# datasciencetoolkit/NextGP.jl

Measured on AMD Instinct MI355X. Metric: gibbs_iterations_per_sec, higher is better.
Workload: dtype f64; 1 GPU; single-trait Gibbs sweep, N=50000 individuals x P=600000 SNPs, marker sets BayesPR(200000) + BayesPR(200000) + BayesPR(200000), fp32 panel in HBM (BASELINE.json configs[3]: multi-breed random regression = three BayesPR marker sets of 200,000 SNPs); N=50000, P=600000, chains=1, panel_dtype=f32, accumulate_dtype=f64

## Files before the change

include/nextgp_hip.h:

```cpp
#ifndef NEXTGP_HIP_H
#define NEXTGP_HIP_H

#include <stdint.h>

#ifdef __cplusplus
extern "C" {
#endif

#define NGP_ABI_VERSION 4

#define NGP_OK 0
#define NGP_ERR_ARG (-1)
#define NGP_ERR_STATE (-2)
#define NGP_ERR_HIP (-3)
#define NGP_ERR_NOMEM (-4)
#define NGP_ERR_NODEVICE (-5)
#define NGP_ERR_DEBUG (-6)

#define NGP_METHOD_BAYESPR 0
#define NGP_METHOD_BAYESB 1
#define NGP_METHOD_BAYESC 2
#define NGP_METHOD_BAYESR 3
#define NGP_METHOD_TUPLE 4
#define NGP_METHOD_BAYESLV 5
// ... 94 lines not shown

int32_t ngp_draws_indexed(ngp_handle *h, uint64_t iter, uint64_t kind, uint64_t index0, int32_t what, double p1, double p2,
                          int64_t n, double *out);
int32_t ngp_eval_math(ngp_handle *h, int32_t which, const double *in, int64_t n, double *out);

int32_t ngp_set_streamer(ngp_handle *h, int32_t variant);
int32_t ngp_get_streamer(ngp_handle *h, int32_t *variant, int32_t *gemv_chains);

int32_t ngp_set_max_shards(ngp_handle *h, int32_t max_shards);
int32_t ngp_shards_for_chains(ngp_handle *h, int32_t chains, int32_t *max_shards);
int32_t ngp_share_panel(ngp_handle *h, ngp_handle *owner);
int32_t ngp_shards_for_pass(ngp_handle *h, int32_t chains, int32_t *max_shards);
#define NGP_STORAGE_F32 0
#define NGP_STORAGE_U8 1
int32_t ngp_set_storage(ngp_handle *h, int32_t storage);
int32_t ngp_get_storage(ngp_handle *h, int32_t *storage, double *means, int64_t P);

int32_t ngp_debug_set_mode(ngp_handle *h, int32_t mode);
int32_t ngp_debug_set_knob(ngp_handle *h, int32_t knob);

int32_t ngp_set_posterior_sums(ngp_handle *h, const double *sum_beta, const double *sum_beta2, const double *sum_delta,
                               const double *sum_varBeta, const double *sum_pi, double sum_varE, double sum_b, int64_t nKept);
int32_t ngp_save_snapshot(ngp_handle *h, const char *path);
int32_t ngp_load_snapshot(ngp_handle *h, const char *path);

int32_t ngp_set_trace_loci(ngp_handle *h, const int64_t *loci, int64_t n, int64_t n_varBeta);
int32_t ngp_get_trace_ext(ngp_handle *h, double *beta_tr, double *varBeta_tr, double *pi_tr, int64_t n);

int32_t ngp_allreduce_posterior(ngp_handle **hs, int32_t n);
int32_t ngp_run_many(ngp_handle **hs, int32_t n, int64_t niter);

int32_t ngp_set_sample_file(ngp_handle *h, const char *path);
int32_t ngp_get_census(ngp_handle *h, uint64_t *out, int64_t n, int64_t *grid, int64_t *retries, int32_t *exclusive);
int32_t ngp_debug_fail_census(ngp_handle *h, int64_t iteration);
int32_t ngp_debug_set_virtual_device(ngp_handle *h, int32_t vdev);
int32_t ngp_debug_throw(ngp_handle *h, int32_t kind);

int32_t ngp_add_marker_set_lv(ngp_handle *h, int64_t col0, int64_t ncol, double varBeta0, const double *C, int64_t ld, int32_t ncov,
                              double varZeta0, int32_t est_mode, double est_fraction, const double *zeta0, const double *lhs0,
                              const double *rhs0, int32_t *set_id);
int32_t ngp_get_lv_state(ngp_handle *h, int32_t set_id, double *c, double *sum_c, double *varZeta, double *sum_varZeta, double *zeta,
                         double *iCpC, int64_t *trapped);
int32_t ngp_set_lv_state(ngp_handle *h, int32_t set_id, const double *c, const double *sum_c, double varZeta, double sum_varZeta,
                         const double *zeta);

int32_t ngp_grm_begin(ngp_handle *h, int64_t N, int32_t method);
int32_t ngp_grm_columns_f64(ngp_handle *h, const double *M, int64_t ncol, int64_t ld);
int32_t ngp_grm_columns_f32(ngp_handle *h, const float *M, int64_t ncol, int64_t ld);
int32_t ngp_grm_columns_u8(ngp_handle *h, const uint8_t *M, int64_t ncol, int64_t ld);
int32_t ngp_grm_end(ngp_handle *h);
int32_t ngp_grm_get(ngp_handle *h, double *G_out);
int32_t ngp_grm_invert(ngp_handle *h);
int32_t ngp_add_random_set_dense(ngp_handle *h, const int32_t *level, int64_t q, const double *K, ngp_handle *k_src, int32_t k_src_set,
                                 double df, double scale, double varU0, int32_t *set_id);
int32_t ngp_set_records(ngp_handle *h, int64_t N);

#ifdef __cplusplus
}
#endif
#endif
```

nextgp.jl_amd/_lib.py:

```python
import ctypes as C
import os

import numpy as np

_HERE = os.path.dirname(os.path.abspath(__file__))
LIB_PATH = os.environ.get("NGP_HIP_LIB") or os.path.join(_HERE, "libnextgp_hip.so")

METHOD_BAYESPR, METHOD_BAYESB, METHOD_BAYESC, METHOD_BAYESR, METHOD_TUPLE, METHOD_BAYESLV = 0, 1, 2, 3, 4, 5
LV_MAXCOV, LV_WORDS = 16, 17


def _sample_header(f, path):
    magic = f.read(8)
    if magic not in (b"NGPSMP01", b"NGPSMP02", b"NGPSMP03"):
        raise NextGPHipError(f"not a sample file: {path}")
    P, nvb, nsets, nfix, ncls, rec = (int(v) for v in np.frombuffer(f.read(48), dtype=np.int64))
    sets = [dict(zip(("method", "K", "col0", "ncol", "nvb", "tk"), np.frombuffer(f.read(48), dtype=np.int64).tolist())) for _ in range(nsets)]
    rq = []
    if magic in (b"NGPSMP02", b"NGPSMP03"):
        nr = int(np.frombuffer(f.read(8), dtype=np.int64)[0])
        rq = np.frombuffer(f.read(8 * nr), dtype=np.int64).tolist()
    lv = []
    if magic == b"NGPSMP03":
        nl = int(np.frombuffer(f.read(8), dtype=np.int64)[0])
# ... 73 lines not shown
    return col0 + 64 * (l // Lb) + k * (l % Lb) + np.arange(k, dtype=np.int64)[None, :]


def tuple_span(nloc, k):
    Lb = 64 // k
    nblk = (nloc + Lb - 1) // Lb
    return 64 * (nblk - 1) + k * (nloc - Lb * (nblk - 1))


def tuple_panel(sets):
    k, (N, nloc) = len(sets), sets[0].shape
    out = np.zeros((N, tuple_span(nloc, k)), dtype=sets[0].dtype, order="F")
    cols = tuple_columns(0, nloc, k)
    for m, X in enumerate(sets):
        out[:, cols[:, m]] = X
    return out

SYMBOLS = [
    "ngp_abi_version", "ngp_create", "ngp_destroy", "ngp_last_error", "ngp_set_panel_f64", "ngp_set_panel_f32", "ngp_set_panel_u8",
    "ngp_begin_panel", "ngp_panel_columns_f64", "ngp_panel_columns_f32", "ngp_panel_columns_u8", "ngp_end_panel",
    "ngp_generate_panel", "ngp_get_layout", "ngp_get_mpm", "ngp_get_gram", "ngp_xbeta", "ngp_add_marker_set", "ngp_set_y",
    "ngp_set_residual_prior", "ngp_set_intercept", "ngp_set_schedule", "ngp_run", "ngp_get_state", "ngp_set_state",
    "ngp_get_trace", "ngp_get_posterior_sums", "ngp_posterior_len", "ngp_export_posterior_device", "ngp_sweep_set", "ngp_sweep_set_dev",
    "ngp_get_timing", "ngp_profile_iteration", "ngp_draws_indexed", "ngp_eval_math", "ngp_configure", "ngp_get_config", "ngp_debug_stamps", "ngp_set_near_lags", "ngp_get_near_lags",
    "ngp_set_streamer", "ngp_get_streamer", "ngp_set_storage", "ngp_get_storage", "ngp_set_max_shards", "ngp_shards_for_chains", "ngp_run_many", "ngp_write_panel_file", "ngp_read_panel_header", "ngp_load_panel_file", "ngp_debug_set_mode", "ngp_debug_set_knob", "ngp_set_posterior_sums", "ngp_save_snapshot", "ngp_load_snapshot",
    "ngp_set_trace_loci", "ngp_get_trace_ext", "ngp_allreduce_posterior", "ngp_add_marker_set_r", "ngp_get_class_state", "ngp_set_class_state", "ngp_add_fixed_set", "ngp_get_fixed", "ngp_set_fixed", "ngp_debug_throw", "ngp_get_census", "ngp_debug_set_virtual_device", "ngp_debug_fail_census", "ngp_add_marker_set_tuple", "ngp_share_panel", "ngp_shards_for_pass", "ngp_set_sample_file",
    "ngp_set_chain_form", "ngp_get_chain_form", "ngp_get_setup_timing", "ngp_set_residual_weights", "ngp_get_residual_weights",
    "ngp_add_random_set", "ngp_get_random", "ngp_set_random", "ngp_sample_random_set",
    "ngp_add_marker_set_lv", "ngp_get_lv_state", "ngp_set_lv_state",
    "ngp_grm_begin", "ngp_grm_columns_f64", "ngp_grm_columns_f32", "ngp_grm_columns_u8", "ngp_grm_end", "ngp_grm_get", "ngp_grm_invert",
    "ngp_add_random_set_dense", "ngp_set_records",
    "ngp_set_random_schedule", "ngp_get_random_schedule", "ngp_pedigree_ainv",
    "ngp_add_random_set_tuple", "ngp_get_random_tuple", "ngp_set_random_tuple", "ngp_sample_random_set_tuple",
]

_lib = None


class NextGPHipError(RuntimeError):
    pass


def load():
    global _lib
    if _lib is None:
        if not os.path.exists(LIB_PATH):
            raise NextGPHipError(
                f"{LIB_PATH} is missing: build it with `python -c 'import __graft_entry__ as g; g.build()'` "
                "(hipcc --offload-arch=gfx950). There is no CPU fallback.")
        L = C.CDLL(LIB_PATH)
        L.ngp_last_error.restype = C.c_char_p
        L.ngp_last_error.argtypes = [C.c_void_p]
        _lib = L
    return _lib


def _p(a, t):
    return a.ctypes.data_as(C.POINTER(t)) if a is not None else None


def write_panel_file(path, G, bits=8):
    G = np.asfortranarray(G, dtype=np.uint8)
    rc = load().ngp_write_panel_file(str(path).encode(), _p(G, C.c_uint8), C.c_int64(G.shape[0]), C.c_int64(G.shape[1]),
                                     C.c_int64(G.shape[0]), C.c_int32(bits))
    if rc != 0:
        raise NextGPHipError(f"ngp_write_panel_file failed ({rc}): path not writable, or codes above 2 with bits=2")
# ... 536 lines not shown
    def set_posterior_sums(self, ps):
        a = {k: np.ascontiguousarray(ps[k], dtype=np.float64) for k in ("sum_beta", "sum_beta2", "sum_delta", "sum_varBeta", "sum_pi")}
        self._chk(self.L.ngp_set_posterior_sums(self.h, _p(a["sum_beta"], C.c_double), _p(a["sum_beta2"], C.c_double),
                                                _p(a["sum_delta"], C.c_double), _p(a["sum_varBeta"], C.c_double), _p(a["sum_pi"], C.c_double),
                                                C.c_double(ps["sum_varE"]), C.c_double(ps["sum_b"]), C.c_int64(ps["nKept"])))

    def set_sample_file(self, path):
        self._chk(self.L.ngp_set_sample_file(self.h, None if path is None else os.fsencode(path)))

    def save_snapshot(self, path):
        self._chk(self.L.ngp_save_snapshot(self.h, os.fsencode(path)))

    def load_snapshot(self, path):
        self._chk(self.L.ngp_load_snapshot(self.h, os.fsencode(path)))

    def set_trace_loci(self, loci, n_varBeta=0):
        loci = np.ascontiguousarray(loci, dtype=np.int64)
        self._chk(self.L.ngp_set_trace_loci(self.h, _p(loci, C.c_int64) if len(loci) else None, C.c_int64(len(loci)), C.c_int64(n_varBeta)))
        self.ntl, self.ntvb = len(loci), n_varBeta

    def get_trace_ext(self, n):
        bt = np.empty((n, max(self.ntl, 1))); vt = np.empty((n, max(self.ntvb, 1))); pt = np.empty((n, max(self.nsets, 1)))
        self._chk(self.L.ngp_get_trace_ext(self.h, _p(bt, C.c_double), _p(vt, C.c_double), _p(pt, C.c_double), C.c_int64(n)))
        return dict(beta=bt[:, :self.ntl], varBeta=vt[:, :self.ntvb], pi=pt[:, :self.nsets])

    def census(self):
        g, r, e = C.c_int64(), C.c_int64(), C.c_int32()
        self._chk(self.L.ngp_get_census(self.h, None, C.c_int64(0), C.byref(g), C.byref(r), C.byref(e)))
        tb = np.zeros(g.value, dtype=np.uint64)
        self._chk(self.L.ngp_get_census(self.h, _p(tb, C.c_uint64), C.c_int64(g.value), None, None, None))
        return dict(grid=g.value, retries=r.value, exclusive=bool(e.value), xcc=(tb >> np.uint64(32)).astype(np.int64) - 1,
                    hw_id=(tb & np.uint64(0xFFFFFFFF)).astype(np.int64))

    def debug_fail_census(self, iteration):
        self._chk(self.L.ngp_debug_fail_census(self.h, C.c_int64(iteration)))

    def debug_set_virtual_device(self, vdev):
        self._chk(self.L.ngp_debug_set_virtual_device(self.h, C.c_int32(vdev)))

    @staticmethod
    def allreduce_posterior(samplers):
        L = samplers[0].L
        arr = (C.c_void_p * len(samplers))(*[s.h for s in samplers])
        samplers[0]._chk(L.ngp_allreduce_posterior(arr, C.c_int32(len(samplers))))

    @staticmethod
    def run_many(samplers, niter):
        L = samplers[0].L
        arr = (C.c_void_p * len(samplers))(*[s.h for s in samplers])
        rc = L.ngp_run_many(arr, C.c_int32(len(samplers)), C.c_int64(niter))
        if rc != 0:
            msgs = [(s.L.ngp_last_error(s.h) or b"").decode() for s in samplers]
            raise NextGPHipError(f"libnextgp_hip error {rc}: " + " | ".join(m for m in msgs if m))

    def profile_iteration(self):
        ms, by = C.c_double(), C.c_double()
        n = C.c_int64()
        self._chk(self.L.ngp_profile_iteration(self.h, C.byref(ms), C.byref(n), C.byref(by)))
        return dict(avg_ms=ms.value, launches=n.value, bytes_per_launch=by.value)

    def draws_indexed(self, it, kind, index0, what, n, p1=0.0, p2=0.0):
        out = np.empty(n)
        self._chk(self.L.ngp_draws_indexed(self.h, C.c_uint64(it), C.c_uint64(kind), C.c_uint64(index0), C.c_int32(what),
                                           C.c_double(p1), C.c_double(p2), C.c_int64(n), _p(out, C.c_double)))
        return out

# ... 6 lines not shown
```

nextgp.jl_amd/csrc/ngp_api.hip:

```cpp
#include <hip/hip_runtime.h>

#include <dlfcn.h>

#include <algorithm>
#include <chrono>
#include <cmath>
#include <cstdio>
#include <cstdlib>
#include <condition_variable>
#include <cstddef>
#include <cstring>
#include <array>
#include <deque>
#include <map>
#include <memory>
#include <mutex>
#include <queue>
#include <string>
#include <thread>
#include <vector>

#include "../../include/nextgp_hip.h"
#include "ngp_kernels.h"
#include "ngp_random.h"
// ... 807 lines not shown
        HCHK(hipMemcpy(h->mm.d_tseg_len, h->h_tseg_len.data(), h->h_tseg_len.size() * sizeof(int32_t), hipMemcpyHostToDevice));
        HCHK(hipMemcpy(h->mm.d_tseg_set, h->h_tseg_set.data(), h->h_tseg_set.size() * sizeof(int32_t), hipMemcpyHostToDevice));
    }
    h->tables_dirty = false;
    return NGP_OK;
}

bool is_kept(const ngp_handle *h, int64_t it) {
    if (it < h->burnIn + h->thin || it > h->chainLength) return false;
    return ((it - h->burnIn) % h->thin) == 0;
}

void fill_sweep_args(ngp_handle *h, int64_t tb0, int64_t tb1, SweepArgs &A) {
    const int R = (int)h->plan.R, S = (int)h->plan.S;
    A.tiles = h->pm->tiles; A.ycorr = h->cm.d_ycorr; A.gramx = h->pm->gramx;
    const bool tf = wants_tinv(h) && h->cm.tinv_blocks == h->NBLK;
    A.tinv = (tf && h->cm.lin_any) ? h->cm.d_tinv : nullptr;
    A.blin = (tf && h->cm.lin_any) ? h->cm.d_blin : nullptr;
    A.lin_all = (tf && h->cm.lin_any) ? h->cm.lin_all : 0;
    A.V = h->plan.V; A.D = h->plan.D; A.R = R; A.S = S; A.NG = h->plan.NG; A.near = h->plan.near; A.fine_ok = 0; A.t0 = (int)tb0; A.t1 = (int)tb1;
    A.beta = h->cm.d_beta; A.delta = h->cm.d_delta; A.c = h->cm.d_c; A.w = h->cm.d_w; A.q = h->cm.d_q; A.mpm = h->pm->mpm; A.chi = h->cm.d_chi;
    A.setof = h->cm.d_setof; A.vbidx = h->cm.d_vbidx; A.sets = h->cm.d_sets; A.varBeta = h->mm.d_varBeta;
    A.rcls = h->mm.d_rcls; A.rhs0 = h->cm.d_rhs0; A.scal = h->cm.d_scal; A.Ppad = h->Ppad;
    A.tup = h->ntuple ? h->mm.d_tup : nullptr; A.tupc = h->mm.d_tupc; A.tupg = h->mm.d_tupg;
    A.acc = (unsigned long long *)h->cm.d_ccnt.get(); A.dlt = h->cm.d_cdlt; A.dltg = h->cm.d_cdltg;
    h->launch_seq = (h->launch_seq % 4095u) + 1u;
    A.nonce = h->launch_seq;
    A.flag_dlt = h->cm.d_ccnt + (size_t)NGP_RING * NGP_FX_COPIES * NGP_BLK * 2; A.abort_w = h->cm.d_abort; A.xcc_w = h->cm.d_abort + 16;
    A.census = (h->dbg_mode == 0) ? h->cm.d_ccnt + h->cm.census_off : nullptr;
    A.census_tbl = h->cm.d_census_tbl; A.iter_tag = (unsigned)(h->iter + 1);
    A.census_fail = (h->dbg_census_fail_iter > 0 && !h->exclusive) ? (unsigned)h->dbg_census_fail_iter : 0u;
    A.dbg = h->hm.d_dbg;
    A.fine_ok = (streamer_lds(h->plan, 1) + 8192 <= sweep_lds(h->plan, SweepKernel::diag)) ? 1 : 0;
    A.variant = h->plan.streamer; A.knob = h->knob;
    A.mean = h->pm->mean; A.N = h->N;
    A.dbg_mode = h->dbg_mode;
}

void launch_sweep(ngp_handle *h, int64_t tb0, int64_t tb1, hipEvent_t *evs) {
    const int R = (int)h->plan.R, S = (int)h->plan.S;
    if (h->plan.mode == 1) {
        SweepArgs A;
        fill_sweep_args(h, tb0, tb1, A);
        const SweepKernel k = pick_kernel(h->plan, 1, h->hm.d_dbg || h->dbg_mode, h->ntuple > 0, h->nclass_total > 0);
        h->last_grid = sweep_grid(h->plan);
        if (evs) (void)hipEventRecord(evs[0], h->stream);
        launch_sweep_kernel(k, h->last_grid, sweep_lds(h->plan, k), h->stream, &A);
        if (evs) (void)hipEventRecord(evs[1], h->stream);
        h->sweep_launches += 1;
        return;
    }
    int e = 0;
    for (int64_t t = tb0; t <= tb1; t++) {
        const int do_upd = t > tb0, do_gemv = t < tb1;
        if (evs && do_gemv) (void)hipEventRecord(evs[e++], h->stream);
        hipLaunchKernelGGL(k_step, dim3((unsigned)S), dim3(256), h->lds_step, h->stream, h->pm->tiles, h->cm.d_ycorr, h->cm.d_dlt, h->cm.d_part, R,
                           S, (int)t, do_upd, do_gemv);
        if (evs && do_gemv) (void)hipEventRecord(evs[e++], h->stream);
        if (do_gemv)
            hipLaunchKernelGGL(k_recur, dim3(1), dim3(256), 0, h->stream, h->cm.d_part, h->pm->gramx, h->plan.D, S, (int)t, h->cm.d_beta, h->cm.d_delta,
                               h->cm.d_c, h->cm.d_w, h->cm.d_q, h->pm->mpm, h->cm.d_chi, h->cm.d_setof, h->cm.d_vbidx, h->cm.d_sets, h->mm.d_varBeta, h->cm.d_dlt, h->mm.d_rcls,
                               (long long)h->Ppad, h->cm.d_rhs0, h->cm.d_scal, h->mm.d_tup, h->mm.d_tupc, h->mm.d_tupg,
                               (const double *)((wants_tinv(h) && h->cm.tinv_blocks == h->NBLK && h->cm.lin_any) ? h->cm.d_tinv : nullptr), (const unsigned *)h->cm.d_blin);
    }
    h->sweep_launches += 2 * (tb1 - tb0) + 1;
}

// ... 2960 lines not shown
    h->smp.reset();
    if (!path) return NGP_OK;
    REQUIRE(h->pm, NGP_ERR_STATE, "panel not set");
    auto S = std::make_unique<SampleStream>();
    S->path = path; S->device = h->device;
    S->f.reset(std::fopen(path, "wb"));
    if (!S->f) return fail(h, NGP_ERR_ARG, std::string("cannot open the sample file for writing: ") + path);
    hipError_t e = hipStreamCreate(&S->copy_stream);
    for (int i = 0; i < SampleStream::NSLOT && e == hipSuccess; i++) {
        e = hipEventCreateWithFlags(&S->ev_packed[i], hipEventDisableTiming);
        if (e == hipSuccess) e = hipEventCreateWithFlags(&S->ev_copied[i], hipEventDisableTiming);
    }
    if (e != hipSuccess) return fail(h, NGP_ERR_HIP, std::string("sample stream: ") + hipGetErrorString(e));
    S->writer = std::thread(sample_writer_loop, S.get());
    h->smp = std::move(S);
    return NGP_OK;
    NGP_CATCH(h)
}

int32_t ngp_get_census(ngp_handle *h, uint64_t *out, int64_t n, int64_t *grid, int64_t *retries, int32_t *exclusive) {
    NGP_TRY
    int rc;
    if ((rc = enter(h))) return rc;
    REQUIRE(h->pm && h->plan.mode == 1, NGP_ERR_STATE, "no persistent sweep on this handle");
    const int64_t g = h->last_grid > 0 ? h->last_grid : sweep_grid(h->plan);
    if (grid) *grid = g;
    if (retries) *retries = h->census_retries;
    if (exclusive) *exclusive = h->exclusive ? 1 : 0;
    if (out) {
        REQUIRE(n >= g, NGP_ERR_ARG, "census buffer smaller than the grid");
        HCHK(hipStreamSynchronize(h->stream));
        HCHK(hipMemcpy(out, h->cm.d_census_tbl, (size_t)g * sizeof(uint64_t), hipMemcpyDeviceToHost));
    }
    return NGP_OK;
    NGP_CATCH(h)
}

int32_t ngp_debug_fail_census(ngp_handle *h, int64_t iteration) {
    NGP_TRY
    int rc;
    if ((rc = enter(h))) return rc;
    REQUIRE(iteration >= 0, NGP_ERR_ARG, "iteration must be >= 0");
    h->dbg_census_fail_iter = iteration;
    if (iteration > 0) h->exclusive = false;
    return NGP_OK;
    NGP_CATCH(h)
}

int32_t ngp_debug_set_virtual_device(ngp_handle *h, int32_t vdev) {
    NGP_TRY
    int rc;
    if ((rc = enter(h))) return rc;
    REQUIRE(vdev >= -1 && vdev < 64, NGP_ERR_ARG, "virtual device: -1 (off) or 0..63");
    h->vdev = vdev;
    return NGP_OK;
    NGP_CATCH(h)
}

int32_t ngp_debug_throw(ngp_handle *h, int32_t kind) {
    NGP_TRY
    if (kind == 0) throw std::bad_alloc();
    if (kind == 1) { std::vector<double> v; v.resize(v.max_size() + 1); }
    if (kind == 2) throw 42;
    return fail(h, NGP_ERR_ARG, "ngp_debug_throw: kind must be 0, 1 or 2");
    NGP_CATCH(h)
}
// ... 290 lines not shown
```

nextgp.jl_amd/csrc/ngp_sweep.h:

```cpp
#pragma once
#include <cstddef>
#include <type_traits>
#include "ngp_sweep_args.h"

#ifndef NGP_ROWS_DPP
#define NGP_ROWS_DPP 1
#endif

#pragma clang fp contract(off)

namespace ngp {


#define NGP_DBG_FOLD                                                     \
    unsigned long long *const dbg = DBG ? A.dbg : nullptr;               \
    const int dbg_mode = DBG ? A.dbg_mode : 0;                           \
    (void)dbg; (void)dbg_mode;
#define NGP_DBG_LOCALS                                                   \
    unsigned long long *const dbg = A.dbg;                               \
    const int dbg_mode = A.dbg_mode;                                     \
    (void)dbg; (void)dbg_mode;
#define NGP_DBG_ROWS NGP_DBG_FOLD

__device__ inline unsigned ld_u32(const unsigned *p) { return __hip_atomic_load(p, __ATOMIC_RELAXED, __HIP_MEMORY_SCOPE_AGENT); }
// ... 101 lines not shown
            return false;
        }
        __builtin_amdgcn_s_sleep(4);
    }
}

__device__ inline void load_rows_pair(const double *blk, int j, double (&out)[NGP_BLK]) {
    const double2 *p = (const double2 *)blk + j;
#pragma unroll
    for (int k2 = 0; k2 < NGP_BLK / 2; k2++) {
        const double2 v = p[k2 * NGP_BLK];
        out[2 * k2] = v.x;
        out[2 * k2 + 1] = v.y;
    }
}

__device__ inline unsigned sld_u32(const unsigned *p) {
    const unsigned long long a = (unsigned long long)p;
    p = (const unsigned *)(((unsigned long long)(unsigned)__builtin_amdgcn_readfirstlane((int)(a >> 32)) << 32) |
                           (unsigned)__builtin_amdgcn_readfirstlane((int)(unsigned)a));
    unsigned v;
    asm volatile("s_load_dword %0, %1, 0x0 glc\n\ts_waitcnt lgkmcnt(0)" : "=s"(v) : "s"(p) : "memory");
    return v;
}

__device__ inline void sld_u32x2(const unsigned *p0, const unsigned *p1, unsigned &v0, unsigned &v1) {
    const unsigned long long a0 = (unsigned long long)p0, a1 = (unsigned long long)p1;
    p0 = (const unsigned *)(((unsigned long long)(unsigned)__builtin_amdgcn_readfirstlane((int)(a0 >> 32)) << 32) |
                            (unsigned)__builtin_amdgcn_readfirstlane((int)(unsigned)a0));
    p1 = (const unsigned *)(((unsigned long long)(unsigned)__builtin_amdgcn_readfirstlane((int)(a1 >> 32)) << 32) |
                            (unsigned)__builtin_amdgcn_readfirstlane((int)(unsigned)a1));
    asm volatile("s_load_dword %0, %2, 0x0 glc\n\ts_load_dword %1, %3, 0x0\n\ts_waitcnt lgkmcnt(0)" : "=&s"(v0), "=&s"(v1) : "s"(p0), "s"(p1) : "memory");
}
__device__ inline const double *chain_block_src(const SweepArgs &A, const long long t, const bool lin) {
    return lin ? A.tinv + (size_t)t * (NGP_BLK * NGP_BLK) : A.gramx + ((size_t)t * A.D + 0) * (NGP_BLK * NGP_BLK);
}
__device__ __attribute__((always_inline)) inline size_t warm_bytes(const SweepArgs &A, const int planes) {
    return (size_t)(planes + ((A.tinv && !A.lin_all) ? 1 : 0)) * (NGP_BLK * NGP_BLK * sizeof(double));
}
__device__ __attribute__((always_inline)) inline size_t warm_t_hi(const SweepArgs &A) { return A.tinv ? (size_t)(NGP_BLK * NGP_BLK * sizeof(double)) : 0; }
__device__ __attribute__((always_inline)) inline size_t warm_shift(const SweepArgs &A) {
    return (A.tinv && !A.lin_all) ? (size_t)(NGP_BLK * NGP_BLK * sizeof(double)) : 0;
}

template <typename GLoad>
__device__ inline double gemv4(GLoad G, const double *d) {
    double s0 = 0.0, s1 = 0.0, s2 = 0.0, s3 = 0.0;
#pragma unroll 16
    for (int k = 0; k < NGP_BLK; k += 4) {
        s0 = __builtin_fma(G(k + 0), d[k + 0], s0);
        s1 = __builtin_fma(G(k + 1), d[k + 1], s1);
        s2 = __builtin_fma(G(k + 2), d[k + 2], s2);
        s3 = __builtin_fma(G(k + 3), d[k + 3], s3);
    }
    return (s0 + s1) + (s2 + s3);
}

template <bool DBG, int DT, int NGP_TPT>
__device__ inline void role_streamer(const SweepArgs &A, const int s, char *smem) {
    NGP_DBG_LOCALS
    const int R = A.R, S = A.S, tid = threadIdx.x;
    const int wv = tid >> 6, j = tid & 63;
    const size_t TB = (size_t)R * 256;
    const size_t TBL = (size_t)(R >> 2) * NGP_QS;
    char *ring = smem;
    constexpr bool FUSE1 = (NGP_TPT == 1);
    double *ys = (double *)(smem + 2 * TBL);
    double *red = ys + 2 * R;
    double *dl = red + 512;
    int *sflag = (int *)(dl + 128);
    char *scratch = (char *)(dl + 128) + 64;
    double *pp = (double *)(scratch + 3072);
    unsigned long long *fine = (unsigned long long *)(pp + 8 * (size_t)R);
    const bool fine_on = dbg && s == 1 && A.fine_ok == 1;
#define NGP_FINE(k)                                                                                          \
    do {                                                                                                     \
        if (fine_on && (unsigned)(u - 800) < 16u && j == 0) fine[(((u - 800) * 8 + wv) << 3) + (k)] = wall_clock64(); \
    } while (0)
    const size_t tile_elems = (size_t)R * NGP_BLK;
    const int nchunk = R >> 2;
    const int ntask = (8 * R + NGP_WG - 1) / NGP_WG;
    double *yg = A.ycorr + (size_t)s * R;
    const int g = s / NGP_GRP;
    const int nb = A.t1 - A.t0;
    auto dma_tile = [&](int ub) {
        if (dbg_mode == 4) return;
        const char *src = (const char *)(A.tiles + ((size_t)(A.t0 + ub) * S + s) * tile_elems);
        char *dst = ring + (size_t)(ub & 1) * TBL;
        for (int c = wv - 4; c < nchunk; c += 3) dma16_lds(src + (size_t)c * 1024 + (size_t)j * 16, dst + (size_t)c * NGP_QS);
    };
    auto poll_dlt = [&](int uu) {
        const int aa = uu - DT;
        if (aa < 0 || uu >= nb + DT) return;
        int ok = 1;
        if (j == 0) {
            ok = (dbg_mode == 3 || dbg_mode == 4 || wait_ge(A.flag_dlt, (unsigned)(aa + 1), A.abort_w, 1u)) ? 1 : 0;
            if (dbg && s == 0) dbg[NGP_DBG_STREAM + 2 * (size_t)uu + 1] = wall_clock64();
            if (!ok) *sflag = 0;
        }
        ok = __builtin_amdgcn_readfirstlane(ok);
        __builtin_amdgcn_fence(__ATOMIC_ACQUIRE, "wavefront");
        if (ok) dl[(uu & 1) * 64 + j] = ld_f64(&A.dlt[(size_t)(aa % NGP_RING) * NGP_BLK + j]);
    };
    const int gpc = R / NGP_TPT;
    const int tq_ = min(tid, 8 * gpc - 1);
    const int tcc = tq_ / gpc, ti0 = (tq_ - tcc * gpc) * NGP_TPT;
    float keep[DT][NGP_TPT][8];
// ... 282 lines not shown
#define NGP_VMC8(b) NGP_VMC(b) NGP_VMC(b + 1) NGP_VMC(b + 2) NGP_VMC(b + 3) NGP_VMC(b + 4) NGP_VMC(b + 5) NGP_VMC(b + 6) NGP_VMC(b + 7)
    switch (n) {
        NGP_VMC(1) NGP_VMC(2) NGP_VMC(3) NGP_VMC(4) NGP_VMC(5) NGP_VMC(6) NGP_VMC(7) NGP_VMC(8) NGP_VMC(9) NGP_VMC(10) NGP_VMC(11)
        NGP_VMC(12) NGP_VMC(13) NGP_VMC(14) NGP_VMC(15) NGP_VMC(16) NGP_VMC(17) NGP_VMC(18) NGP_VMC(19) NGP_VMC(20) NGP_VMC(21)
        NGP_VMC(22) NGP_VMC(23) NGP_VMC(24) NGP_VMC(25) NGP_VMC(26) NGP_VMC(27) NGP_VMC(28) NGP_VMC(29) NGP_VMC(30) NGP_VMC(31)
        NGP_VMC(32) NGP_VMC(33) NGP_VMC(34) NGP_VMC(35) NGP_VMC(36) NGP_VMC(37) NGP_VMC(38) NGP_VMC(39) NGP_VMC(40) NGP_VMC(41)
        NGP_VMC(42) NGP_VMC(43) NGP_VMC(44) NGP_VMC(45) NGP_VMC(46) NGP_VMC(47) NGP_VMC(48) NGP_VMC(49) NGP_VMC(50) NGP_VMC(51)
        NGP_VMC(52) NGP_VMC(53) NGP_VMC(54) NGP_VMC(55) NGP_VMC(56) NGP_VMC(57) NGP_VMC(58) NGP_VMC(59) NGP_VMC(60) NGP_VMC(61)
        NGP_VMC(62) NGP_VMC(63)
        default: asm volatile("s_waitcnt vmcnt(0)" ::: "memory"); break;
    }
#undef NGP_VMC8
#undef NGP_VMC
}

template <bool DBG, int DT, int ST>
__device__ __attribute__((always_inline)) inline void role_streamer_rows(const SweepArgs &A, const int s, char *smem) {
    NGP_DBG_ROWS
    constexpr bool U8 = (ST != 0);
    constexpr int NT = U8 ? ST : 1;
    const int R = A.R, S = A.S, tid = threadIdx.x;
    const int wv = __builtin_amdgcn_readfirstlane(tid >> 6), lane = tid & 63;
    const int NQ = U8 ? (R >> 4) : (R >> 2);
    const int H = min(NGP_ROWS_HMAX, (NQ + 1) >> 1);
    const int RQ = 2 * NQ + H;
    char *ring = smem;
    double *ys = (double *)(smem + (size_t)RQ * NGP_QS);
    double *red = ys + ((R + 7) & ~7);
    double *dl = red + 2 * NGP_ROWS_NW * NGP_BLK;
    double *rsy = dl + 2 * NGP_DLS;
    int *sflag = (int *)(rsy + 16);
    char *scratch = (char *)(rsy + 16) + 64;
    unsigned long long *fine = (unsigned long long *)(scratch + 1024);
    const bool fine_on = DBG && dbg && s == 1 && A.fine_ok == 1;
#define NGP_FINE(k)                                                                                              \
    do {                                                                                                         \
        if (fine_on && (unsigned)(u - 800) < 16u && lane == 0) fine[(((u - 800) * 8 + wv) << 3) + (k)] = wall_clock64(); \
    } while (0)
    const size_t tile_bytes = (size_t)NQ * 1024;
    double *yg = A.ycorr + (size_t)s * R;
    const int g = s / NGP_GRP;
    const int nb = A.t1 - A.t0;
    for (int i = tid; i < R; i += NGP_WG) ys[i] = yg[i];
    int *gcnt0 = (int *)(rsy + 7), *gcnt1 = (int *)(rsy + 15);
    const bool early = U8 ? ((A.knob & 256) != 0) : ((A.knob & 256) == 0);
    if (tid == 0) { *sflag = 1; *gcnt0 = 0; *gcnt1 = 0; }
    int base = 0;
    auto wrap = [&](int p) __attribute__((always_inline)) { return p >= RQ ? p - RQ : p; };
    if (wv == NGP_ROWS_NW) {
        const unsigned ring0 = (unsigned)(size_t)(__attribute__((address_space(3))) const char *)ring;
        const unsigned scratch0 = (unsigned)(size_t)(__attribute__((address_space(3))) const char *)scratch;
        const unsigned voff = (unsigned)lane * 16u;
        const bool no_dma = DBG && dbg_mode == 4;
        const int pace = A.knob & 7;
        auto dma_quads = [&](int tile, int q0, int q1, int tbase) __attribute__((always_inline)) {
            if (no_dma || q0 >= q1) return 0;
            const char *g = (const char *)A.tiles + ((size_t)(A.t0 + tile) * S + s) * tile_bytes + (size_t)q0 * 1024;
            int p = wrap(tbase + q0);
            int q = q0;
            for (; q + 4 <= q1; q += 4) {
                if (p + 4 <= RQ) {
                    dma16_s4(ring0 + (unsigned)p * NGP_QS, g, voff);
                    p += 4;
                    if (p == RQ) p = 0;
                    switch (pace) {
                        case 1: __builtin_amdgcn_s_sleep(1); break;
                        case 2: __builtin_amdgcn_s_sleep(2); break;
// ... 1 lines not shown
                        case 4: __builtin_amdgcn_s_sleep(4); break;
                        default: break;
                    }
                } else {
                    for (int k = 0; k < 4; k++) {
                        dma16_s(ring0 + (unsigned)p * NGP_QS, g + k * 1024, voff);
                        if (++p == RQ) p = 0;
                    }
                }
                g += 4096;
            }
            for (; q < q1; ++q) {
                dma16_s(ring0 + (unsigned)p * NGP_QS, g, voff);
                g += 1024;
                if (++p == RQ) p = 0;
            }
            return q1 - q0;
        };
        const unsigned my_xcc = xcc_id() + 1u;
        const int nslice = max(1, S / 8);
        const int slice = (s / 8) % nslice;
        const size_t gram_bytes = warm_bytes(A, min(DT, A.near + 1)), w_thi = warm_t_hi(A), w_shift = warm_shift(A);
        const size_t slice_bytes = ((gram_bytes / nslice + 1023) / 1024) * 1024;
        bool same_xcd = false, xcc_known = false;
        __builtin_amdgcn_s_setprio(3);
        if (nb > 0) dma_quads(0, 0, NQ, 0);
        if (nb > 1) dma_quads(1, 0, H, NQ);
        drain_vm();
        wg_barrier();
        for (int u = 0; u < nb + DT; ++u) {
            NGP_FINE(0);
            const int base1 = wrap(base + NQ), base2 = wrap(base1 + NQ);
            if (!xcc_known && (u & 7) == 0) {
                const unsigned x = sld_u32(A.xcc_w);
                xcc_known = (x != 0u);
                same_xcd = (x == my_xcc);
            }
            if (same_xcd && u + 1 < nb && !no_dma) {
                const char *gb = (const char *)(A.gramx + (size_t)(A.t0 + u + 1) * DT * NGP_BLK * NGP_BLK) - w_shift;
                const char *tb = (const char *)(A.tinv + (size_t)(A.t0 + u + 1) * NGP_BLK * NGP_BLK);
                const size_t lo = (size_t)slice * slice_bytes, hi = min((size_t)(slice + 1) * slice_bytes, gram_bytes);
                for (size_t off = lo; off + 1024 <= hi; off += 1024) dma16_warm(scratch0, (off < w_thi ? tb : gb) + off, voff);
            }
            if (u + 1 < nb) dma_quads(u + 1, H, NQ, base1);
            int n2 = 0;
            if (u + 2 < nb) n2 = dma_quads(u + 2, 0, H, base2);
            NGP_FINE(1);
            wait_vmcnt_le(n2);
            NGP_FINE(2);
            wg_barrier();
            if (!*sflag) return;
            base = base1;
        }
        drain_vm();
    } else {
        const int c = lane & 7, ql = lane >> 3;
        const int nqw = (NQ - wv + NGP_ROWS_NW - 1) / NGP_ROWS_NW;
        int tslot[NT], trow[NT];
        bool thas[NT];
#pragma unroll
        for (int i = 0; i < NT; i++) {
            if constexpr (U8) {
                const int tau = ql + 8 * i;
                thas[i] = (tau >> 2) < nqw;
                tslot[i] = thas[i] ? wv + NGP_ROWS_NW * (tau >> 2) : wv;
                trow[i] = 16 * tslot[i] + 4 * (tau & 3);
            } else {
                const int qt = wv + NGP_ROWS_NW * ql;
                thas[i] = qt < NQ;
// ... 487 lines not shown
            {
                const unsigned long long *gp = A.dltg + ((size_t)(a % NGP_RING) * NGP_BLK + lane) * 2;
                q0 = ld_u64(gp);
                q1 = ld_u64(gp + 1);
            }
            if (!(dbg_mode == 3 || dbg_mode == 4 || dbg_mode == 6) && !wait_dlt_granules_all(A.dltg, A.nonce, a, lane, A.abort_w, 4u, q0, q1)) return;
            const double dreg = dlt_granules_value(q0, q1);
            double *ldw = (double *)smem + (size_t)wv * NGP_BLK;
            ldw[lane] = dreg;
            typedef const __attribute__((address_space(3))) double *lds_cdp;
            const lds_cdp dk = (lds_cdp)ldw;
            double s0 = 0.0, s1 = 0.0, s2 = 0.0, s3 = 0.0;
#pragma unroll
            for (int kk = 0; kk < NGP_BLK; kk += 16) {
                double dv[16];
#pragma unroll
                for (int i = 0; i < 16; i++) dv[i] = dk[kk + i];
#pragma unroll
                for (int i = 0; i < 16; i += 4) {
                    s0 = __builtin_fma(gr[kk + i + 0], dv[i + 0], s0);
                    s1 = __builtin_fma(gr[kk + i + 1], dv[i + 1], s1);
                    s2 = __builtin_fma(gr[kk + i + 2], dv[i + 2], s2);
                    s3 = __builtin_fma(gr[kk + i + 3], dv[i + 3], s3);
                }
                asm volatile("" : "+v"(s0), "+v"(s1), "+v"(s2), "+v"(s3));
            }
            const double v = (s0 + s1) + (s2 + s3);
            acc_add(A.acc, A.abort_w, slot, d, lane, -v, fxs);
            if (dbg && g == 0 && lane == 0) dbg[NGP_DBG_RED + 2 * (size_t)u + 1] = wall_clock64();
        }
    }
}

struct CoefRegs {
    double bo, cc, ww, st, gd;
    unsigned tf;
};
__device__ inline CoefRegs load_coef(const SweepArgs &A, long long k) {
    CoefRegs c;
    c.bo = A.beta[k];
    c.cc = A.c[k];
    c.ww = A.w[k];
    c.st = A.q[k];
    c.gd = A.mpm[k];
    c.tf = A.lin_all ? 1u : (A.blin ? A.blin[k >> 6] : 0u);
    return c;
}
__device__ __attribute__((always_inline)) inline unsigned acc_terms(const SweepArgs &A, const int u) {
    const int nfar = max(0, min(A.D - 1, u) - A.near);
    return (unsigned)(A.S + nfar);
}
__device__ __attribute__((always_inline)) inline unsigned long long acc_load(const SweepArgs &A, const int u, const int j) {
    const unsigned long long *ap = A.acc + (size_t)(u % NGP_RING) * NGP_FX_COPIES * NGP_BLK + j;
    unsigned long long qv[NGP_FX_COPIES];
#pragma unroll
    for (int c = 0; c < NGP_FX_COPIES; c++) qv[c] = ld_u64(ap + (size_t)c * NGP_BLK);
    unsigned long long q = qv[0];
#pragma unroll
    for (int c = 1; c < NGP_FX_COPIES; c++) q += qv[c];
    return q;
}
__device__ __attribute__((always_inline)) inline bool acc_complete(const unsigned long long q, const unsigned terms) {
    return __ballot((unsigned)(q & ((1ull << NGP_FX_CNT_BITS) - 1ull)) == terms) == ~0ull;
}
__device__ __attribute__((always_inline)) inline void acc_zero(const SweepArgs &A, const int u, const int j) {
    unsigned long long *ap = A.acc + (size_t)(u % NGP_RING) * NGP_FX_COPIES * NGP_BLK + j;
// ... 1397 lines not shown
```

nextgp.jl_amd/csrc/ngp_sweep_args.h:

```cpp
#pragma once
#include "ngp_common.h"

#define NGP_RING 16
#define NGP_MAX_LAG 12
#define NGP_SPIN_LIMIT (1u << 21)
#define NGP_WG 512
#define NGP_DBG_WAVES (1u << 19)
#define NGP_DBG_RED (3u << 18)
#define NGP_DBG_W5 (5u << 17)
#define NGP_DBG_ALL (7u << 17)
#define NGP_DBG_RELOOK (NGP_DBG_ALL - 3)
#define NGP_SPARSE_MAX 16
#ifndef NGP_LAZY_LAG
#define NGP_LAZY_LAG 7
#endif
#define NGP_QS 1040
#define NGP_SAMPLER_TUPLE_LDS (2 * 9 * 64 * 8 + 64)
#define NGP_SAMPLER_R_LDS (2 * 17 * 64 * 8 + 2 * 128 * 4 + 64 + 2 * 16 * 64 * 8)
#define NGP_ABORT_CENSUS 9u
#define NGP_CENSUS_TICKS 2000000ull
#define NGP_DBG_STREAM (1u << 20)

namespace ngp {

struct SweepArgs {
    const float *tiles;
    double *ycorr;
    const double *gramx;
    const double *tinv;
    const unsigned *blin;
    int lin_all;
    int knob;
    int variant;
    int V;
    int D, R, S, NG, near, fine_ok, t0, t1;
    double *beta;
    uint8_t *delta;
    const double *c, *w, *q, *mpm, *chi;
    const int8_t *setof;
    const int32_t *vbidx;
    DSet *sets;
    double *varBeta;
    const double *rcls;
    const double *rhs0;
    const DScal *scal;
    long long Ppad;
    const DTup *tup;
    const double *tupc, *tupg;
    const double *mean;
    long long N;
    unsigned long long *acc;
    double *dlt;
    unsigned long long *dltg;
    unsigned nonce;
// ... 63 lines not shown
```

nextgp.jl_amd/csrc/ngp_sweep_body.inc:

```
    extern __shared__ __attribute__((aligned(16))) char smem[];
    NGP_DBG_LOCALS
    const int b = blockIdx.x;
    if (ld_u32(A.abort_w) != 0u) return;
    if (!sweep_census(A, b, smem)) return;
    if (dbg_mode == 1 && b <= A.NG) return;
    if ((dbg_mode == 2 && b != 0) || ((dbg_mode == 3 || dbg_mode == 4) && b == 0)) return;
    if (b == 0)
        role_sampler<DBG, false, TUP, RCLSV>(A, smem);
    else if (b <= A.NG)
        role_reducer<DBG>(A, b - 1, smem);
    else {
        const int s = b - 1 - A.NG;
        if (A.variant == 2) {
            switch (A.D) {
                case 3: role_streamer_rows<DBG, 3, 0>(A, s, smem); break;
                case 4: role_streamer_rows<DBG, 4, 0>(A, s, smem); break;
                case 5: role_streamer_rows<DBG, 5, 0>(A, s, smem); break;
                default: role_streamer_rows<DBG, 6, 0>(A, s, smem); break;
            }
            return;
        }
        if (A.variant == 3) {
            const int nt = ngp_u8_tasks(A.R);
            if (nt == 1) {
                switch (A.D) {
                    case 3: role_streamer_rows<DBG, 3, 1>(A, s, smem); break;
                    case 4: role_streamer_rows<DBG, 4, 1>(A, s, smem); break;
                    case 6: role_streamer_rows<DBG, 6, 1>(A, s, smem); break;
                    case 8: role_streamer_rows<DBG, 8, 1>(A, s, smem); break;
                    default: role_streamer_rows<DBG, 12, 1>(A, s, smem); break;
                }
            } else if (nt == 2) {
                if (A.D == 4) role_streamer_rows<DBG, 4, 2>(A, s, smem);
                else role_streamer_rows<DBG, 8, 2>(A, s, smem);
            } else {
                role_streamer_rows<DBG, 4, 4>(A, s, smem);
            }
            return;
        }
        const int tpt = (8 * A.R + NGP_WG - 1) / NGP_WG;
#define NGP_DISPATCH_D(T)                                      \
    switch (A.D) {                                             \
        case 1: role_streamer<DBG, 1, T>(A, s, smem); break;        \
        case 2: role_streamer<DBG, 2, T>(A, s, smem); break;        \
// ... 25 lines not shown
```

Baseline: 43.59 it/s.

## Repurpose an idle reducer block as an L2 cache warmer for row streaming

Adds a warmer role. When the plan uses the rows streamer with tall R and the reducer count leaves one reducer idle, the last reducer block runs this role instead of reducing. The warmer waits for the sampler's XCD id; if it shares that XCD, it prefetches upcoming gram/tinv blocks into cache via DMA, staying a fixed distance behind sampler progress. The f32 streamer then skips its own same-XCD prefetch when the warmer has taken over. This risks losing a reducer's work and adds extra polling and cache traffic.

```diff
diff --git a/include/nextgp_hip.h b/include/nextgp_hip.h
--- a/include/nextgp_hip.h
+++ b/include/nextgp_hip.h
@@ -150,6 +150,7 @@
 
 int32_t ngp_set_sample_file(ngp_handle *h, const char *path);
 int32_t ngp_get_census(ngp_handle *h, uint64_t *out, int64_t n, int64_t *grid, int64_t *retries, int32_t *exclusive);
+int32_t ngp_get_warmer(ngp_handle *h, int32_t *active, int64_t *blocks);
 int32_t ngp_debug_fail_census(ngp_handle *h, int64_t iteration);
 int32_t ngp_debug_set_virtual_device(ngp_handle *h, int32_t vdev);
 int32_t ngp_debug_throw(ngp_handle *h, int32_t kind);
diff --git a/nextgp.jl_amd/_lib.py b/nextgp.jl_amd/_lib.py
--- a/nextgp.jl_amd/_lib.py
+++ b/nextgp.jl_amd/_lib.py
@@ -129,6 +129,7 @@
     "ngp_add_random_set_dense", "ngp_set_records",
     "ngp_set_random_schedule", "ngp_get_random_schedule", "ngp_pedigree_ainv",
     "ngp_add_random_set_tuple", "ngp_get_random_tuple", "ngp_set_random_tuple", "ngp_sample_random_set_tuple",
+    "ngp_get_warmer",
 ]
 
 _lib = None
@@ -731,6 +732,11 @@
         return dict(grid=g.value, retries=r.value, exclusive=bool(e.value), xcc=(tb >> np.uint64(32)).astype(np.int64) - 1,
                     hw_id=(tb & np.uint64(0xFFFFFFFF)).astype(np.int64))
 
+    def warmer(self):
+        a, b = C.c_int32(), C.c_int64()
+        self._chk(self.L.ngp_get_warmer(self.h, C.byref(a), C.byref(b)))
+        return dict(active=a.value, blocks=b.value)
+
     def debug_fail_census(self, iteration):
         self._chk(self.L.ngp_debug_fail_census(self.h, C.c_int64(iteration)))
 
diff --git a/nextgp.jl_amd/csrc/ngp_api.hip b/nextgp.jl_amd/csrc/ngp_api.hip
--- a/nextgp.jl_amd/csrc/ngp_api.hip
+++ b/nextgp.jl_amd/csrc/ngp_api.hip
@@ -863,7 +863,11 @@
     A.census_fail = (h->dbg_census_fail_iter > 0 && !h->exclusive) ? (unsigned)h->dbg_census_fail_iter : 0u;
     A.dbg = h->hm.d_dbg;
     A.fine_ok = (streamer_lds(h->plan, 1) + 8192 <= sweep_lds(h->plan, SweepKernel::diag)) ? 1 : 0;
-    A.variant = h->plan.streamer; A.knob = h->knob;
+    const bool warmer_tall = h->plan.R >= NGP_WARMER_MIN_R || (h->knob & NGP_KNOB_WARMER_ANY_R);
+    const bool warmer_idle = h->plan.NG > 0 && h->plan.NG % 8 == 0 && h->plan.near + h->plan.NG >= h->plan.D;
+    const bool warmer = h->dbg_mode == 0 && h->plan.streamer == 2 && h->plan.V == 1 && !(h->knob & NGP_KNOB_NO_WARMER) &&
+                        warmer_tall && warmer_idle;
+    A.variant = h->plan.streamer; A.knob = (h->knob & ~NGP_KNOB_WARMER) | (warmer ? NGP_KNOB_WARMER : 0);
     A.mean = h->pm->mean; A.N = h->N;
     A.dbg_mode = h->dbg_mode;
 }
@@ -3890,6 +3894,20 @@
         HCHK(hipStreamSynchronize(h->stream));
         HCHK(hipMemcpy(out, h->cm.d_census_tbl, (size_t)g * sizeof(uint64_t), hipMemcpyDeviceToHost));
     }
+    return NGP_OK;
+    NGP_CATCH(h)
+}
+
+int32_t ngp_get_warmer(ngp_handle *h, int32_t *active, int64_t *blocks) {
+    NGP_TRY
+    int rc;
+    if ((rc = enter(h))) return rc;
+    REQUIRE(h->pm && h->plan.mode == 1, NGP_ERR_STATE, "no persistent sweep on this handle");
+    unsigned w[3] = {0, 0, 0};
+    HCHK(hipStreamSynchronize(h->stream));
+    HCHK(hipMemcpy(w, h->cm.d_ccnt + h->cm.census_off + 8, sizeof(w), hipMemcpyDeviceToHost));
+    if (active) *active = w[1] ? 1 : 0;
+    if (blocks) *blocks = (int64_t)w[2];
     return NGP_OK;
     NGP_CATCH(h)
 }
diff --git a/nextgp.jl_amd/csrc/ngp_sweep.h b/nextgp.jl_amd/csrc/ngp_sweep.h
--- a/nextgp.jl_amd/csrc/ngp_sweep.h
+++ b/nextgp.jl_amd/csrc/ngp_sweep.h
@@ -157,6 +157,14 @@
                             (unsigned)__builtin_amdgcn_readfirstlane((int)(unsigned)a1));
     asm volatile("s_load_dword %0, %2, 0x0 glc\n\ts_load_dword %1, %3, 0x0\n\ts_waitcnt lgkmcnt(0)" : "=&s"(v0), "=&s"(v1) : "s"(p0), "s"(p1) : "memory");
 }
+__device__ inline void sld_u32x2_glc(const unsigned *p0, const unsigned *p1, unsigned &v0, unsigned &v1) {
+    const unsigned long long a0 = (unsigned long long)p0, a1 = (unsigned long long)p1;
+    p0 = (const unsigned *)(((unsigned long long)(unsigned)__builtin_amdgcn_readfirstlane((int)(a0 >> 32)) << 32) |
+                            (unsigned)__builtin_amdgcn_readfirstlane((int)(unsigned)a0));
+    p1 = (const unsigned *)(((unsigned long long)(unsigned)__builtin_amdgcn_readfirstlane((int)(a1 >> 32)) << 32) |
+                            (unsigned)__builtin_amdgcn_readfirstlane((int)(unsigned)a1));
+    asm volatile("s_load_dword %0, %2, 0x0 glc\n\ts_load_dword %1, %3, 0x0 glc\n\ts_waitcnt lgkmcnt(0)" : "=&s"(v0), "=&s"(v1) : "s"(p0), "s"(p1) : "memory");
+}
 __device__ inline const double *chain_block_src(const SweepArgs &A, const long long t, const bool lin) {
     return lin ? A.tinv + (size_t)t * (NGP_BLK * NGP_BLK) : A.gramx + ((size_t)t * A.D + 0) * (NGP_BLK * NGP_BLK);
 }
@@ -166,6 +174,11 @@
 __device__ __attribute__((always_inline)) inline size_t warm_t_hi(const SweepArgs &A) { return A.tinv ? (size_t)(NGP_BLK * NGP_BLK * sizeof(double)) : 0; }
 __device__ __attribute__((always_inline)) inline size_t warm_shift(const SweepArgs &A) {
     return (A.tinv && !A.lin_all) ? (size_t)(NGP_BLK * NGP_BLK * sizeof(double)) : 0;
+}
+__device__ __attribute__((always_inline)) inline unsigned *warmer_words(const SweepArgs &A) { return A.flag_dlt + 40; }
+__device__ __attribute__((always_inline)) inline int fine_shard(const SweepArgs &A) {
+    const int f = (A.knob >> 16) & 0xfff;
+    return f ? f - 1 : 1;
 }
 
 template <typename GLoad>
@@ -197,7 +210,7 @@
     char *scratch = (char *)(dl + 128) + 64;
     double *pp = (double *)(scratch + 3072);
     unsigned long long *fine = (unsigned long long *)(pp + 8 * (size_t)R);
-    const bool fine_on = dbg && s == 1 && A.fine_ok == 1;
+    const bool fine_on = dbg && s == (DBG ? fine_shard(A) : 1) && A.fine_ok == 1;
 #define NGP_FINE(k)                                                                                          \
     do {                                                                                                     \
         if (fine_on && (unsigned)(u - 800) < 16u && j == 0) fine[(((u - 800) * 8 + wv) << 3) + (k)] = wall_clock64(); \
@@ -546,7 +559,7 @@
     int *sflag = (int *)(rsy + 16);
     char *scratch = (char *)(rsy + 16) + 64;
     unsigned long long *fine = (unsigned long long *)(scratch + 1024);
-    const bool fine_on = DBG && dbg && s == 1 && A.fine_ok == 1;
+    const bool fine_on = DBG && dbg && s == (DBG ? fine_shard(A) : 1) && A.fine_ok == 1;
 #define NGP_FINE(k)                                                                                              \
     do {                                                                                                         \
         if (fine_on && (unsigned)(u - 800) < 16u && lane == 0) fine[(((u - 800) * 8 + wv) << 3) + (k)] = wall_clock64(); \
@@ -614,9 +627,17 @@
             NGP_FINE(0);
             const int base1 = wrap(base + NQ), base2 = wrap(base1 + NQ);
             if (!xcc_known && (u & 7) == 0) {
-                const unsigned x = sld_u32(A.xcc_w);
-                xcc_known = (x != 0u);
-                same_xcd = (x == my_xcc);
+                if constexpr (U8) {
+                    const unsigned x = sld_u32(A.xcc_w);
+                    xcc_known = (x != 0u);
+                    same_xcd = (x == my_xcc);
+                } else {
+                    unsigned x, wx = 0u;
+                    if (A.knob & NGP_KNOB_WARMER) sld_u32x2_glc(A.xcc_w, warmer_words(A), x, wx);
+                    else x = sld_u32(A.xcc_w);
+                    xcc_known = (x != 0u) && (x != my_xcc || !(A.knob & NGP_KNOB_WARMER) || wx != 0u);
+                    same_xcd = (x == my_xcc) && (wx != x) && !(A.knob & NGP_KNOB_NO_WARM);
+                }
             }
             if (same_xcd && u + 1 < nb && !no_dma) {
                 const char *gb = (const char *)(A.gramx + (size_t)(A.t0 + u + 1) * DT * NGP_BLK * NGP_BLK) - w_shift;
@@ -1170,6 +1191,57 @@
     }
 }
 
+#ifndef NGP_WARM_DIST
+#define NGP_WARM_DIST 1
+#endif
+#define NGP_WARMER_DECLINED 0xFFu
+template <bool DBG>
+__device__ __attribute__((always_inline)) inline void role_warmer(const SweepArgs &A, char *smem) {
+    NGP_DBG_LOCALS
+    const int tid = threadIdx.x, lane = tid & 63;
+    const int wv = __builtin_amdgcn_readfirstlane(tid >> 6);
+    const int nb = A.t1 - A.t0, DT = A.D;
+    unsigned *ww = warmer_words(A);
+    const unsigned my_xcc = xcc_id() + 1u;
+    unsigned x = 0u;
+    for (unsigned spins = 0; spins < (1u << 14); ++spins) {
+        x = ld_u32(A.xcc_w);
+        if (x != 0u) break;
+        if ((spins & 31u) == 31u && ld_u32(A.abort_w) != 0u) break;
+        __builtin_amdgcn_s_sleep(8);
+    }
+    const bool warms = (x == my_xcc);
+    if (tid == 0) {
+        if (warms) st_u32(ww + 1, 1u);
+        st_u32(ww, warms ? my_xcc : NGP_WARMER_DECLINED);
+    }
+    if (!warms) return;
+    const unsigned sink = (unsigned)(size_t)(__attribute__((address_space(3))) const char *)(smem + wv * 1024);
+    const unsigned voff = (unsigned)lane * 16u;
+    const size_t gram_bytes = warm_bytes(A, min(DT, A.near + 1)), w_thi = warm_t_hi(A), w_shift = warm_shift(A);
+    unsigned done = 0u;
+    for (int t = wv; t < nb; t += NGP_WG / 64) {
+        const int a = t - DT - NGP_WARM_DIST;
+        if (a >= 0) {
+            const unsigned long long *gp = A.dltg + (size_t)(a % NGP_RING) * NGP_BLK * 2;
+            bool ok = false;
+            for (unsigned spins = 0; spins <= (NGP_SPIN_LIMIT >> 3); ++spins) {
+                const unsigned tag = (unsigned)(ld_u64(gp) >> 32);
+                if ((tag >> 20) == A.nonce && (tag & 0xFFFFFu) >= (unsigned)(a + 1)) { ok = true; break; }
+                if ((spins & 7u) == 7u && ld_u32(A.abort_w) != 0u) break;
+                __builtin_amdgcn_s_sleep(2);
+            }
+            if (!ok) break;
+        }
+        const char *gb = (const char *)(A.gramx + (size_t)(A.t0 + t) * DT * NGP_BLK * NGP_BLK) - w_shift;
+        const char *tb = (const char *)(A.tinv + (size_t)(A.t0 + t) * NGP_BLK * NGP_BLK);
+        for (size_t off = 0; off + 1024 <= gram_bytes; off += 1024) dma16_warm(sink, (off < w_thi ? tb : gb) + off, voff);
+        ++done;
+    }
+    drain_vm();
+    if (lane == 0 && done) atomicAdd(ww + 2, done);
+}
+
 struct CoefRegs {
     double bo, cc, ww, st, gd;
     unsigned tf;
diff --git a/nextgp.jl_amd/csrc/ngp_sweep_args.h b/nextgp.jl_amd/csrc/ngp_sweep_args.h
--- a/nextgp.jl_amd/csrc/ngp_sweep_args.h
+++ b/nextgp.jl_amd/csrc/ngp_sweep_args.h
@@ -20,6 +20,11 @@
 #define NGP_ABORT_CENSUS 9u
 #define NGP_CENSUS_TICKS 2000000ull
 #define NGP_DBG_STREAM (1u << 20)
+#define NGP_KNOB_NO_WARM 2048
+#define NGP_KNOB_WARMER 4096
+#define NGP_KNOB_NO_WARMER 8192
+#define NGP_KNOB_WARMER_ANY_R 16384
+#define NGP_WARMER_MIN_R 160
 
 namespace ngp {
 
diff --git a/nextgp.jl_amd/csrc/ngp_sweep_body.inc b/nextgp.jl_amd/csrc/ngp_sweep_body.inc
--- a/nextgp.jl_amd/csrc/ngp_sweep_body.inc
+++ b/nextgp.jl_amd/csrc/ngp_sweep_body.inc
@@ -7,9 +7,10 @@
     if ((dbg_mode == 2 && b != 0) || ((dbg_mode == 3 || dbg_mode == 4) && b == 0)) return;
     if (b == 0)
         role_sampler<DBG, false, TUP, RCLSV>(A, smem);
-    else if (b <= A.NG)
-        role_reducer<DBG>(A, b - 1, smem);
-    else {
+    else if (b <= A.NG) {
+        if (b == A.NG && (A.knob & NGP_KNOB_WARMER)) role_warmer<DBG>(A, smem);
+        else role_reducer<DBG>(A, b - 1, smem);
+    } else {
         const int s = b - 1 - A.NG;
         if (A.variant == 2) {
             switch (A.D) {
```

New measurement: 47.28 it/s, median of 6. 1.08x the previous value.
